# daihangpku/SW-NeRF

Measured on AMD Instinct MI355X. Metric: rays/sec (64+128 samples/ray), higher is better.
Workload: dtype f32

## Files before the change

### include/swnerf.h

```cpp
#ifndef SWNERF_H
#define SWNERF_H
#include <stddef.h>
#include <stdint.h>

#ifdef __cplusplus
extern "C" {
#endif

#define SWNERF_VERSION 112

#define SWNERF_E_ARG      (-1)
#define SWNERF_E_UNSUPP   (-2)

#define SWNERF_NET_CANON   0
#define SWNERF_NET_DNERF   1
#define SWNERF_NET_NOVIEW  2
#define SWNERF_NET_TNERF   3


int         swnerf_version(void);
const char* swnerf_last_error(void);

size_t swnerf_packed_floats(int kind);
int swnerf_pack_net(int kind, const float* const* params , int L_pos, int L_dir,
// ... 244 lines not shown
                         int64_t* count);
void swnerf_adam_caps(int* max_tensors, int* max_blocks, int64_t* chunk, size_t* descriptor_bytes);

#define SWNERF_PATCH_MAX_LEVELS 4
#define SWNERF_PATCH_MAX_SIDE   32
#define SWNERF_MULTIRES_LOSSES  11
int swnerf_patch_batch(int n_levels, const float* const* pyr_images , const int* level_hw , const double* focal ,
                       const int* corner , const int* patch , const float* images, int64_t n_images, const float* c2w,
                       const float* times, int64_t img_i, double near, double far, float* const* ray_batches ,
                       float* const* targets , float* full_patch, void* stream);
int swnerf_multires_loss(int n_levels, const int* patch_hw , const float* const* rgb ,
                         const float* const* rgb0 , const float* const* targets , const float* full_patch,
                         int add_global, float* losses, float* reconstructed, float* const* d_rgb ,
                         float* const* d_rgb0 , void* stream);

#ifdef __cplusplus
}
#endif
#endif
```

### sw-nerf_amd/csrc/pack_kernels.hip

```cpp
#include <hip/hip_runtime.h>
#include "../../include/swnerf.h"
#include "swnerf_common.h"
#include "host_util.h"

enum { KT_TRUNK = 0, KT_POS0 = 1, KT_POS1 = 2, KT_DIR = 3, KT_TIME = 4 };

struct PackSeg {
    const float* W; const float* b;
    float* dstW; float* dstB;
    int out_dim, in_dim;
    short NT, KT;
    short transpose, rowmap;
    int row0, kvalid;
    int max_steps;
    short kind;
    unsigned char ktype[10];
    short kbase[10];
};

#define PACK_MAX_SEGS 26
struct PackPlan { int n, Lp, Ld, Lt; int first_block[PACK_MAX_SEGS + 1]; PackSeg seg[PACK_MAX_SEGS]; };
static_assert(sizeof(PackPlan) <= 3800, "a pack plan must fit the kernel-argument segment");

__global__ void __launch_bounds__(256) pack_plan_kernel(PackPlan P) {
// ... 333 lines not shown
extern "C" int swnerf_pack_net_noview(const float* const* params, int L_pos, int out_ch, float* packed, void* stream) {
    if (!params || !packed) return sw_fail(SWNERF_E_ARG, "pack_net_noview: NULL pointer");
    if (L_pos < 0 || L_pos > 10) return sw_fail(SWNERF_E_UNSUPP, "pack_net_noview: %d position bands exceed 10", L_pos);
    if (out_ch < 4 || out_ch > SW_NOVIEW_MAX_OUT)
        return sw_fail(SWNERF_E_UNSUPP, "pack_net_noview: output_ch %d (the reference builds 4 or 5, nerf/run.py:231)", out_ch);
    for (int i = 0; i < 18; ++i) if (!params[i]) return sw_fail(SWNERF_E_ARG, "pack_net_noview: params[%d] is NULL", i);
    hipStream_t st = (hipStream_t)stream;
    Packer pk(st, packed, packed + SW_NOVIEW_W_FLOATS, L_pos, 0, 0);
    pk.trunk(params, params[16], params[17], out_ch, 3 * (1 + 2 * L_pos), 0);
    if (!pk.rc && (pk.w != packed + (size_t)SW_NOVIEW_STEPS * SW_STEP_FLOATS || pk.b != packed + SW_NOVIEW_W_FLOATS + SW_NOVIEW_BIAS_TILES(out_ch) * SW_BIAS_TILE_FLOATS))
        return sw_fail(SWNERF_E_ARG, "pack_net_noview: internal layout mismatch");
    pk.tail();
    return pk.flush();
}

extern "C" size_t swnerf_packed_bwd_floats_kind(int bwd_kind) {
    switch (bwd_kind) {
        case SWNERF_BWD_CANON: return (size_t)SW_BWD_FLOATS;
        case SWNERF_BWD_CANON_INPUT_GRAD: return (size_t)SW_BWD_IG_FLOATS;
        case SWNERF_BWD_DEFORM: return (size_t)SW_DBWD_FLOATS;
        case SWNERF_BWD_DNERF_FUSED: return (size_t)SW_BWD_DN_FLOATS;
    }
    return 0;
}

extern "C" int swnerf_pack_net_bwd_kind(int bwd_kind, const float* const* params, int L_pos, int L_dir, float* packed_bwd, void* stream) {
    if (!params || !packed_bwd) return sw_fail(SWNERF_E_ARG, "pack_net_bwd: NULL pointer");
    if (bwd_kind != SWNERF_BWD_CANON && bwd_kind != SWNERF_BWD_CANON_INPUT_GRAD && bwd_kind != SWNERF_BWD_DEFORM && bwd_kind != SWNERF_BWD_DNERF_FUSED)
        return sw_fail(SWNERF_E_ARG, "pack_net_bwd: unknown stream kind %d", bwd_kind);
    if (L_pos < 0 || L_pos > 10 || L_dir < 0 || L_dir > 4) return sw_fail(SWNERF_E_UNSUPP, "pack_net_bwd: embedder bands (%d,%d) exceed (10,4)", L_pos, L_dir);
// ... 64 lines not shown
```

### sw-nerf_amd/csrc/render_kernels.hip

```cpp
#include <hip/hip_runtime.h>
#include "../../include/swnerf.h"
#include "swnerf_common.h"
#include "mlp_core.h"
#include "host_util.h"
#include "mlp_kernels.h"

#include "render_pass.h"

struct QueryDev {
    const float* pts; int64_t M; const float* dirs; int64_t V; int shared;
    const float* w0; const float* b0; int nbias; const float* wvl; float* out;
};

__global__ void __launch_bounds__(256, 1) query_points_kernel(QueryDev P) {
    extern __shared__ __attribute__((aligned(16))) float lds_bias[];
    const int lane = threadIdx.x & 63, j = lane & 31, h = lane >> 5;
    const int wv = __builtin_amdgcn_readfirstlane(threadIdx.x >> 6);
    float* lds_ring = lds_bias + SW_LDS_BIAS_FLOATS + wv * SW_LDS_RING_FLOATS;
    float* lds_emb = lds_ring + SW_RING * SW_STEP_FLOATS;
    const int64_t tile = (int64_t)blockIdx.x * 4 + wv;
    bias_to_lds(lds_bias, P.b0, P.nbias);
    if (tile * 32 >= P.M) return;
    const int64_t row = tile * 32 + j;
    const bool live = row < P.M;
// ... 18 lines not shown
        ws.base = reinterpret_cast<const char*>(P.wvl);
        canon_tail_rows(in, demb, hv, lds_bias + h * 16, ws);
        float c3[3];
        head_valu<3, 4>(hv, ws, c3);
        sr += c3[0] + hb_rgb[1]; sg += c3[1] + hb_rgb[2]; sb += c3[2] + hb_rgb[3];
    }
    if (live && h == 0) {
        const float inv = 1.f / (float)nv;
        f32x4 r4 = {sr * inv, sg * inv, sb * inv, head[0]};
        *reinterpret_cast<f32x4*>(P.out + row * 4) = r4;
    }
}

int sw_tnerf_render_launch(const swnerf_pass_args& a, hipStream_t st);

extern "C" int swnerf_render_pass(const swnerf_pass_args* args, void* stream) {
    static const PassAccepts accepts = {"render_pass", {SW_COLS(11) | SW_COLS(12), SW_COLS(11) | SW_COLS(12), SW_COLS(8), ~0u },
        SWNERF_E_ARG, "%s: ray_batch must have 11 or 12 columns (use_viewdirs) or 8 (SWNERF_NET_NOVIEW), got %d for kind %d", true, 0};
    if (!args) return sw_fail(SWNERF_E_ARG, "render_pass: NULL args");
    const swnerf_pass_args& a = *args;
    if (a.kind < 0 || a.kind > SWNERF_NET_TNERF) return sw_fail(SWNERF_E_ARG, "unknown net kind %d", a.kind);
    int rc = pass_check(accepts, a);
    if (rc) return rc;
    if (a.kind == SWNERF_NET_TNERF) return sw_tnerf_render_launch(a, (hipStream_t)stream);
    const bool noview = a.kind == SWNERF_NET_NOVIEW;
    if (a.kind == SWNERF_NET_DNERF && a.cols != 12) return sw_fail(SWNERF_E_ARG, "render_pass: D-NeRF needs the frame_time column");
    if (noview && a.dx) return sw_fail(SWNERF_E_ARG, "render_pass: a static net has no position_delta output here");
    PassDev P = pass_dev(a);
    rc = noview ? stream_ptrs_noview(a.packed, a.out_ch, &P.w0, &P.b0, &P.nbias, &P.two_pass)
                : stream_ptrs(a.kind, a.packed, a.run_deform, &P.w0, &P.b0, &P.nbias, &P.two_pass);
    if (rc) return rc;
    P.dir_steps = noview ? 0 : SW_STEPS_DIR;
    P.time_steps = (a.kind == SWNERF_NET_DNERF && P.two_pass) ? SW_STEPS_TIME : 0;
    size_t lds = SW_LDS_FIXED_FLOATS * sizeof(float);
    if ((rc = pass_resampling(accepts.name, a, P, lds))) return rc;
    if (a.n_rays == 0) return 0;
    if (P.time_steps) {
        P.tb_off = (int)(lds / sizeof(float));
        lds += 4 * SW_TB_LDS_FLOATS * sizeof(float);
    }
    const dim3 grid((unsigned)((a.n_rays + 3) / 4)), block(256);
    hipStream_t st = (hipStream_t)stream;
    pass_startup_args(P, grid.x, noview ? SW_NOVIEW_STEPS : (a.kind == SWNERF_NET_DNERF && P.two_pass ? SW_DEFORM_STEPS + SW_CANON_STEPS : SW_CANON_STEPS));
    if (noview) hipLaunchKernelGGL((render_pass_kernel<false, false, 0, false>), grid, block, lds, st, P);
    else if (a.kind == SWNERF_NET_DNERF) hipLaunchKernelGGL(render_pass_kernel<true>, grid, block, lds, st, P);
    else {
        if (a.dx) {
            rc = sw_check(hipMemsetAsync(a.dx, 0, (size_t)a.n_rays * a.n_samples * 3 * sizeof(float), st), "render_pass dx fill");
            if (rc) return rc;
        }
        hipLaunchKernelGGL(render_pass_kernel<false>, grid, block, lds, st, P);
    }
    return sw_check(hipGetLastError(), "render_pass launch");
}

__global__ void __launch_bounds__(256) sample_coarse_kernel(swnerf_pass_args a, float* z_out, float* pts) {
    const int64_t idx = (int64_t)blockIdx.x * 256 + threadIdx.x;
    const int S = a.n_samples;
    if (idx >= a.n_rays * S) return;
    const int64_t ray = idx / S;
    const int s = (int)(idx - ray * S);
    const float* rb = a.ray_batch + ray * a.cols;
    const float z = z_sample(a, ray, rb[6], rb[7], s);
    z_out[idx] = z;
    if (pts) {
        pts[idx * 3 + 0] = rb[0] + rb[3] * z;
        pts[idx * 3 + 1] = rb[1] + rb[4] * z;
        pts[idx * 3 + 2] = rb[2] + rb[5] * z;
// ... 101 lines not shown
```

### sw-nerf_amd/csrc/render_pass.h

```cpp
#pragma once
#include <cstdlib>
#include "mlp_kernels.h"
#include "mlp_core_x3.h"
#include "resample.h"
#include "composite.h"

#define SW_LDS_SC 256
#define SW_LDS_SORT 1024
#define SW_LDS_WAVE_FLOATS (3 * SW_LDS_SC + SW_LDS_SORT)

struct PassDev {
    swnerf_pass_args a;
    const float* w0;
    const float* b0;
    int nbias;
    int two_pass;
    int sort_n, sort_s;
    float* act;
    float* bits;
    float* xs;
    float* act_d; float* bits_d; float* xs_d;
    int dir_steps;
    int time_steps;
    int tb_off;
    int warm_steps;
    int warm_blocks;
    int skew_mode;
    int skew_unit;
};

__device__ __forceinline__ float wave32_sum(float v) {
#pragma unroll
    for (int o = 16; o > 0; o >>= 1) v += __shfl_xor(v, o, 32);
    return v;
}

__device__ __forceinline__ float z_linear(const swnerf_pass_args& a, float near, float far, int s) {
    const float t = sw_linspace(0.f, 1.f, a.n_samples, s);
    if (!a.lindisp) return near * (1.f - t) + far * t;
    return 1.f / (1.f / near * (1.f - t) + 1.f / far * t);
}

__device__ __forceinline__ float z_sample(const swnerf_pass_args& a, int64_t ray, float near, float far, int s) {
// ... 171 lines not shown
    float* lds = PREC ? lds_all + X3Lds<DNERF>::FIXED + wv * SW_LDS_WAVE_FLOATS
                      : lds_all + PassLds<DNERF, TRAIN>::FIXED + wv * SW_LDS_WAVE_FLOATS;
    float* zc = lds;
    float* wc = lds + SW_LDS_SC;
    float* cdf = lds + 2 * SW_LDS_SC;
    float* srt = lds + 3 * SW_LDS_SC;

    const int S = a.n_samples;
    const bool resample = a.n_importance > 0;
    const float* rb = a.ray_batch + ray * a.cols;
    const float ox = rb[0], oy = rb[1], oz = rb[2], dx = rb[3], dy = rb[4], dz = rb[5];
    const float near = rb[6], far = rb[7];
    const float ft = (a.cols == 12) ? rb[8] : 0.f;
    const float v0 = VIEWS ? rb[a.cols - 3] : 0.f, v1 = VIEWS ? rb[a.cols - 2] : 0.f, v2 = VIEWS ? rb[a.cols - 1] : 0.f;
    const float dnorm = sqrtf(dx * dx + dy * dy + dz * dz);

    WStream ws;
    XStream xs;
    if constexpr (PREC != 0) {
        if (!DNERF) {
            f32x16 demb;
            pe_dir(v0, v1, v2, h, demb);
            tile_park(lds_dir, lane, demb);
        }
        x3_start(xs, reinterpret_cast<const char*>(P.w0), lds_bias, lds_ring, lane, wv);
    } else {
        ws_start(ws, P.w0, lds_bias, lds_ring, lane);
        if constexpr (VIEWS) {
            f32x16 demb;
            pe_dir(v0, v1, v2, h, demb);
            if constexpr (TRAIN) tile_park(lds_dir, lane, demb);
            view_bias_tile(demb, lds_vb, lane, ws);
        }
        if constexpr (DNERF) {
            if (P.time_steps) time_bias_tile(ft, h, lds_all + P.tb_off + wv * SW_TB_LDS_FLOATS, lane, ws);
        }
    }

    const float* zrow = a.z_vals ? a.z_vals + ray * S : nullptr;
    const float* zslot = PREC ? lds_x3w + X3Lds<DNERF>::DIR : lds_emb + SW_EMB_LDS_FLOATS;
    const unsigned zslot_addr = __builtin_amdgcn_readfirstlane((unsigned)(size_t)zslot);
    float pr = 0.f, pg = 0.f, pb = 0.f, pd = 0.f, pa = 0.f;
    double Tc = 1.0;
    const int ntiles = (S + 31) >> 5;
#pragma nounroll
    for (int tile = 0; tile < ntiles; ++tile) {
        const int s = tile * 32 + j;
// ... 118 lines not shown
            head[1] = 0.f; head[2] = 0.f;
            x3_canon_pipe<PREC>(px, py, pz, h, lds_dir, lane, head[0], rgb, xs);
            x3_rewind(xs, SW_X3_CANON_CHUNKS, lds_bias, lane);
        } else if constexpr (!VIEWS) {
            trunk_pass<false, false, false, true>(emb, lds_emb, 0.f, false, h, in, out, head, ws);
            float o5[5] = {0.f, 0.f, 0.f, 0.f, 0.f};
            const int nout = (a.out_ch == 5 && !a.raw) ? 4 : a.out_ch;
            head_valu_rt<8>(in, ws, nout, o5);
            ws.bias += (a.out_ch - nout) * 8 * SW_BIAS_TILE_FLOATS;
            rgb[0] = o5[0] + ws.bias[0]; rgb[1] = o5[1] + ws.bias[1]; rgb[2] = o5[2] + ws.bias[2];
            head[0] = o5[3] + ws.bias[3]; head[1] = 0.f; head[2] = 0.f;
            extra = o5[4] + ws.bias[4];
        } else {
            trunk_pass<false>(emb, lds_emb, 0.f, false, h, in, out, head, ws);
        }
        if (!TRAIN && PREC == 0 && VIEWS) canon_tail(in, lds_vb, rgb, ws.bias - SW_BIAS_TILE_FLOATS, ws);
        if constexpr (PREC == 0)
            ws_rewind(ws, P.w0 + (P.dir_steps + P.time_steps) * SW_STEP_FLOATS,
                      lds_bias + ((P.dir_steps ? SW_DIR_BIAS_TILES : 0) + (P.time_steps ? 8 : 0)) * SW_BIAS_TILE_FLOATS, lane);

        const float c0 = rgb[0], c1 = rgb[1], c2 = rgb[2];
        float sg = head[0];
        if (a.raw && live && h == 0) {
            if (!VIEWS && a.out_ch == 5) {
                float* o = a.raw + (ray * S + s) * 5;
                o[0] = c0; o[1] = c1; o[2] = c2; o[3] = sg; o[4] = extra;
            } else {
                f32x4 r4 = {c0, c1, c2, sg};
                *reinterpret_cast<f32x4*>(a.raw + (ray * S + s) * 4) = r4;
            }
        }
        if (a.noise) sg += a.noise[ray * S + sc];
        const float alpha = comp_alpha(sg, comp_dist(s + 1 < S, zn, z, dnorm), live);
        const float w = alpha * comp_transmittance(excl_cumprod_shfl<32>(comp_survival(alpha), j), Tc);
        if (live) {
            if (a.weights && h == 0) a.weights[ray * S + s] = w;
            if (a.z_out && h == 0) a.z_out[ray * S + s] = z;
            if (resample && h == 0) { zc[s] = z; wc[s] = w; }
        }
        comp_accumulate(w, c0, c1, c2, z, pr, pg, pb, pd, pa);
    }

    pr = wave32_sum(pr); pg = wave32_sum(pg); pb = wave32_sum(pb);
    pd = wave32_sum(pd); pa = wave32_sum(pa);
    if (lane == 0 && !ghost) comp_write_maps(pr, pg, pb, pd, pa, a.white_bkgd, ray, a.rgb_map, a.disp_map, a.acc_map, a.depth_map);
    if (!resample || ghost) return;

    wave_lds_sync();
    const int Ni = a.n_importance;
    const double sm = wave_sample_pdf(wc + 1, S - 1, MidBins{zc}, a.u ? a.u + ray * Ni : nullptr, Ni, cdf, srt, lane);
    if (a.z_std) {
        const float sd = wave_zstd(sm, srt, Ni, lane);
        if (lane == 0) a.z_std[ray] = sd;
    }
    wave_rank_merge(zc, S, P.sort_s, srt, Ni, P.sort_n, a.z_fine + ray * (S + Ni), lane);
}
```

### sw-nerf_amd/csrc/swnerf_common.h

```cpp
#pragma once
#include <math.h>
#include <stdint.h>

#if defined(__HIPCC__)
#define SW_HD __host__ __device__ __forceinline__
#else
#define SW_HD static inline
#endif

#define SW_STEP_FLOATS 256
#ifndef SW_RING
#define SW_RING 8
#endif
#define SW_TAIL 16
#define SW_BIAS_TILE_FLOATS 32

#define SW_STEPS_EMB    64
#define SW_STEPS_EMB_T  96
#define SW_STEPS_TIME   32
#define SW_STEPS_TRUNK  256
#define SW_STEPS_VIEWS  144
#define SW_STEPS_DIR    16
#define SW_STEPS_VIEWSH 128
#define SW_CANON_MAIN_STEPS (SW_STEPS_EMB + 4 * SW_STEPS_TRUNK + SW_STEPS_TRUNK + SW_STEPS_EMB + \
// ... 10 lines not shown
#define SW_NOVIEW_STEPS (SW_STEPS_EMB + 4 * SW_STEPS_TRUNK + SW_STEPS_TRUNK + SW_STEPS_EMB + 2 * SW_STEPS_TRUNK)
#define SW_NOVIEW_MAX_OUT 5
#define SW_NOVIEW_BIAS_TILES(out_ch) (64 + 8 * (out_ch) + 1)
#define SW_NOVIEW_W_FLOATS ((SW_NOVIEW_STEPS + SW_TAIL) * SW_STEP_FLOATS)
#define SW_NOVIEW_FLOATS (SW_NOVIEW_W_FLOATS + SW_NOVIEW_BIAS_TILES(SW_NOVIEW_MAX_OUT) * SW_BIAS_TILE_FLOATS)

#define SW_CANON_W_FLOATS   ((SW_CANON_STEPS + SW_TAIL) * SW_STEP_FLOATS)
#define SW_CANON_VL_OFFSET  (SW_CANON_W_FLOATS + SW_CANON_BIAS_TILES * SW_BIAS_TILE_FLOATS)
#define SW_CANON_VL_FLOATS  ((SW_STEPS_VIEWS + SW_TAIL) * SW_STEP_FLOATS)
#define SW_CANON_FOLD_OFFSET (SW_CANON_VL_OFFSET + SW_CANON_VL_FLOATS)
#define SW_CANON_FLOATS     (SW_CANON_FOLD_OFFSET + SW_FOLD_FLOATS)
#define SW_DNERF_W_FLOATS   ((SW_DEFORM_STEPS + SW_CANON_STEPS + SW_TAIL) * SW_STEP_FLOATS)
#define SW_DNERF_A_FLOATS   (SW_DNERF_W_FLOATS + (SW_DEFORM_BIAS_TILES + SW_CANON_BIAS_TILES) * SW_BIAS_TILE_FLOATS)
#define SW_DNERF_FLOATS     (SW_DNERF_A_FLOATS + SW_CANON_FLOATS)

#define SW_ACT_LD    2432
#define SW_ACT_HV    2304
#define SW_BWD_STEPS (16 + 128 + 7 * 256)
#define SW_BWD_W_FLOATS ((SW_BWD_STEPS + SW_TAIL) * SW_STEP_FLOATS)
#define SW_BWD_BIAS_TILES 8
#define SW_BWD_FLOATS (SW_BWD_W_FLOATS + SW_BWD_BIAS_TILES * SW_BIAS_TILE_FLOATS + SW_FOLD_FLOATS)
#define SW_BWD_IG_STEPS (SW_BWD_STEPS + 2 * 64)
#define SW_BWD_IG_W_FLOATS ((SW_BWD_IG_STEPS + SW_TAIL) * SW_STEP_FLOATS)
#define SW_BWD_IG_FLOATS (SW_BWD_IG_W_FLOATS + SW_BWD_BIAS_TILES * SW_BIAS_TILE_FLOATS + SW_FOLD_FLOATS)
#define SW_BWD_DN_STEPS (SW_BWD_IG_STEPS + 7 * 256)
#define SW_BWD_DN_W_FLOATS ((SW_BWD_DN_STEPS + SW_TAIL) * SW_STEP_FLOATS)
#define SW_BWD_DN_FLOATS (SW_BWD_DN_W_FLOATS + (SW_BWD_BIAS_TILES + 24) * SW_BIAS_TILE_FLOATS + SW_FOLD_FLOATS)
#define SW_DBWD_STEPS (7 * 256)
#define SW_DBWD_W_FLOATS ((SW_DBWD_STEPS + SW_TAIL) * SW_STEP_FLOATS)
#define SW_DBWD_BIAS_TILES 24
// ... 132 lines not shown
```

### sw-nerf_amd/swnerf/model.py

```python
import os
import torch
import torch.nn as nn
import torch.nn.functional as F
import numpy as np

from . import _lib, packing
from .embedder import img2mse, mse2psnr, to8b

_CANON_ORDER = ([f"pts_linears.{i}.{p}" for i in range(8) for p in ("weight", "bias")]
                + [f"{n}.{p}" for n in ("views_linears.0", "feature_linear", "alpha_linear", "rgb_linear")
                   for p in ("weight", "bias")])
_NOVIEW_ORDER = ([f"pts_linears.{i}.{p}" for i in range(8) for p in ("weight", "bias")]
                 + [f"output_linear.{p}" for p in ("weight", "bias")])
_DEFORM_ORDER = ([f"_time.{i}.{p}" for i in range(8) for p in ("weight", "bias")]
                 + [f"_time_out.{p}" for p in ("weight", "bias")])


def _bands(ch, d):
    if ch % d:
        return None
    q = ch // d - 1
    return q // 2 if q >= 0 and q % 2 == 0 else None


# ... 173 lines not shown
        buf = packing.pack_weights(self._pack_cache, "noview", _named(self, names), lambda L: L.swnerf_packed_floats(_lib.NET_NOVIEW),
                                   lambda L, arr, buf, st: L.swnerf_pack_net_noview(arr, Lp, out_ch, buf, st), "pack_net_noview")
        return buf, Lp, out_ch

    def packed_bwd_noview(self):
        names, Lp, out_ch = self._noview_params()
        return packing.pack_weights(self._pack_cache, "bwd_noview", _named(self, names), lambda L: L.swnerf_packed_bwd_noview_floats(),
                                    lambda L, arr, buf, st: L.swnerf_pack_net_bwd_noview(arr, Lp, out_ch, buf, st), "pack_net_bwd_noview")

    def packed(self):
        kind, names, Lp, Ld, Lt = self._pack_params()
        buf = packing.pack_weights(self._pack_cache, "fwd", _named(self, names), lambda L: L.swnerf_packed_floats(kind),
                                   lambda L, arr, buf, st: L.swnerf_pack_net(kind, arr, Lp, Ld, Lt, buf, st), "pack_net")
        return kind, buf, Lp, Ld, Lt

    def packed_x3(self):
        kind, packed, Lp, Ld, Lt = self.packed()
        buf = packing.pack_weights(self._pack_cache, "x3", _named(self, self._pack_params()[1]), lambda L: L.swnerf_packed_x3_floats_kind(kind),
                                   lambda L, arr, buf, st: L.swnerf_pack_net_x3_kind(kind, arr, Lp, Ld, Lt, _lib.ptr(packed), buf, st),
                                   "pack_net_x3")
        return buf, Lp, Ld

    def _forward_hip(self, x, t_emb=None, run_deform=0, want_dx=False):
        kind, packed, Lp, Ld, Lt = self.packed()
        x = _lib.dev_f32(x, "x", self.input_ch + self.input_ch_views)
        lead = x.shape[:-1]
        flat = x.reshape(-1, x.shape[-1])
        M = flat.shape[0]
        out = torch.empty((M, 4), dtype=torch.float32, device=x.device)
        dx = torch.empty((M, 3), dtype=torch.float32, device=x.device) if want_dx else None
# ... 205 lines not shown
```

### sw-nerf_amd/swnerf/parallel.py

```python
import os

import torch
import torch.distributed as dist

from .synth import shard_range


def gather_pixels(local, counts=None, group=None, force=False, async_op=False):
    if not (dist.is_available() and dist.is_initialized()):
        if force:
            raise RuntimeError("swnerf.parallel.gather_pixels(force=True) needs an initialised process group")
        return (local, None) if async_op else local
    if dist.get_world_size(group) == 1 and not force:
        return (local, None) if async_op else local
    world = dist.get_world_size(group)
    n, c = local.shape
    if counts is None:
        counts = [n] * world
    if all(k == counts[0] for k in counts):
        out = torch.empty((world * n, c), dtype=local.dtype, device=local.device)
        work = dist.all_gather_into_tensor(out, local.contiguous(), group=group, async_op=async_op)
        return (out, work) if async_op else out
    if async_op:
        raise ValueError("swnerf.parallel.gather_pixels: async_op needs equal shards")
# ... 25 lines not shown
    from . import render as _r, render_dnerf as _rd
    from .ray import get_rays_range
    n_streams = FRAME_STREAMS if streams is None else int(streams)

    def one(ray0, n):
        if frame_time is None:
            o, d = get_rays_range(H, W, K, c2w, ray0, n, device)
            rgb, disp, acc, _ = _r.render(H, W, K, chunk=chunk, rays=(o, d), **render_kwargs)
        else:
            focal = float(K[0][0]) if not isinstance(K, float) else K
            o, d = get_rays_range(H, W, focal, c2w, ray0, n, device)
            rgb, disp, acc, _ = _rd.render(H, W, focal, chunk=chunk, rays=(o, d), frame_time=frame_time, **render_kwargs)
        return torch.cat([rgb, disp[:, None], acc[:, None]], -1)

    def render_range(ray0, n):
        with torch.no_grad():
            dev = torch.device(device) if device is not None else None
            if n_streams <= 1 or n < 8192 or dev is None or dev.type != "cuda":
                return one(ray0, n)
            main = torch.cuda.current_stream(dev)
            if not any(p_.is_cuda for net in (render_kwargs.get("network_fn"), render_kwargs.get("network_fine")) if net is not None
                       for p_ in net.parameters()):
                return one(ray0, n)
            _r.prepack(render_kwargs.get("network_fn"), render_kwargs.get("network_fine"))
            key = (dev.index, n_streams)
            if key not in _FRAME_SIDE:
                _FRAME_SIDE[key] = [torch.cuda.Stream(device=dev) for _ in range(n_streams)]
            side = _FRAME_SIDE[key]
            ev0 = torch.cuda.Event()
            ev0.record(main)
            outs, a = [], 0
# ... 109 lines not shown
```

### sw-nerf_amd/swnerf/render.py

```python
import inspect
import os

import numpy as np
import torch

from . import _lib
from .ray import get_rays, sample_pdf, raw2outputs
from .embedder import EmbedFn, to8b
from .png import write_png
from .model import vallina_NeRF, NeRFOriginal, DirectTemporalNeRF

DEBUG = False
PASS_HOOK = None
Z_TAP = None


def batchify(fn, chunk):
    if chunk is None:
        return fn

    def ret(inputs):
        return torch.cat([fn(inputs[i:i + chunk]) for i in range(0, inputs.shape[0], chunk)], 0)
    return ret

# ... 72 lines not shown
_PRECISIONS = {"fp32": 0, "bf16x3": 3, "bf16x3-fine": 3, "bf16": 1}
_WARNED = {}
PRECISION = os.environ.get("SWNERF_PRECISION", "fp32")
if PRECISION not in _PRECISIONS:
    raise ValueError(f"swnerf: SWNERF_PRECISION={PRECISION!r} is not one of {sorted(_PRECISIONS)}")


def set_precision(name):
    global PRECISION
    if name not in _PRECISIONS:
        raise ValueError(f"swnerf.render.set_precision: unknown precision {name!r} (one of {sorted(_PRECISIONS)})")
    prev, PRECISION = PRECISION, name
    return prev


def prepack(*nets):
    for net in nets:
        if net is None or not hasattr(net, "packed"):
            continue
        if isinstance(net, vallina_NeRF) and net._noview_params() is not None:
            net.packed_noview()
        elif net._is_fused_arch():
            net.packed()
            if _PRECISIONS[PRECISION]:
                net.packed_x3()


def pass_args(rb, kind, packed, bands, S, out_ch, run_deform, inputs, outputs, n_importance=0, *, lindisp=False,
              white_bkgd=False, who="render_pass"):
    N, cols = rb.shape
    Ni = int(n_importance)
    a = _lib.PassArgs()
    a.ray_batch, a.n_rays, a.cols, a.kind, a.packed = rb.data_ptr(), N, cols, kind, packed.data_ptr()
    a.run_deform, (a.L_pos, a.L_dir, a.L_time), a.n_samples, a.out_ch = int(bool(run_deform)), bands, S, out_ch
    a.lindisp, a.white_bkgd, a.n_importance = int(bool(lindisp)), int(bool(white_bkgd)), Ni
    keep = [rb, packed]
    for name, t in inputs.items():
        if t is not None:
            t = _lib.dev_f32(t, name, Ni if name == "u" else S)
            if t.shape[0] != N:
                raise ValueError(f"swnerf.{who}: {name} must have {N} rows, got {tuple(t.shape)}")
            keep.append(t)
            setattr(a, name, t.data_ptr())
    shapes = {"rgb_map": (N, 3), "disp_map": (N,), "acc_map": (N,), "depth_map": (N,), "weights": (N, S), "raw": (N, S, out_ch),
              "dx": (N, S, 3), "z_out": (N, S), "z_fine": (N, S + Ni), "z_std": (N,)}
    out = {k: torch.empty(shapes[k], dtype=torch.float32, device=rb.device) for k in list(outputs) + (["z_fine", "z_std"] if Ni > 0 else [])}
    for k, t in out.items():
        setattr(a, k, t.data_ptr())
    return a, out, keep


def render_pass(ray_batch, net, n_samples, *, z_vals=None, lindisp=False, t_rand=None, noise=None, white_bkgd=False,
                want=("rgb_map", "disp_map", "acc_map"), n_importance=0, u=None, run_deform=True, precision=None):
    noview = isinstance(net, vallina_NeRF) and net._noview_params() is not None
    out_ch = 4
    if noview:
        packed, Lp, out_ch = net.packed_noview()
        kind, Ld, Lt, terms = _lib.NET_NOVIEW, 0, 0, 0
        if _PRECISIONS[PRECISION if precision is None else precision] and not _WARNED.get("noview_x3"):
            _WARNED["noview_x3"] = True
            import warnings
            warnings.warn(f"swnerf: precision {PRECISION if precision is None else precision!r} was requested, but the bf16 paths are built for the "
                          "nets WITH view directions only - this use_viewdirs=False net renders in fp32 (label your numbers accordingly)")
    else:
        kind, packed, Lp, Ld, Lt = net.packed()
        mode = PRECISION if precision is None else precision
        terms = _PRECISIONS[mode]
        if mode == "bf16x3-fine" and n_importance > 0:
            terms = 0
        if terms:
            packed, _, _ = net.packed_x3()
    rb = _lib.dev_f32(ray_batch, "ray_batch")
    N, S = rb.shape[0], int(n_samples)
    a, out, _keep = pass_args(rb, kind, packed, (Lp, Ld, Lt), S, out_ch, run_deform, dict(z_vals=z_vals, t_rand=t_rand, noise=noise, u=u),
                              want, n_importance, lindisp=lindisp, white_bkgd=white_bkgd)
    if PASS_HOOK is not None:
        PASS_HOOK("begin", N, S)
    if terms:
        _lib.check(_lib.lib().swnerf_render_pass_x3(a, terms, _lib.stream_of(rb)), "render_pass_x3")
    else:
        _lib.check(_lib.lib().swnerf_render_pass(a, _lib.stream_of(rb)), "render_pass")
    if PASS_HOOK is not None:
        PASS_HOOK("end", N, S)
    return out


def chunked_backward(rb, act_rows, div, widths, launch, gemm_jobs, rest_on_main=True):
    from .wgrad import _Fan, _chunk_gemms
    N = rb.shape[0]
    rows_per_ray = act_rows // N
    chunk = max(4, (TRAIN_BWD_CHUNK_ROWS // div // rows_per_ray) // 4 * 4)
    bufs = [torch.empty((min(N, chunk) * rows_per_ray, w), dtype=torch.float32, device=rb.device) for w in widths]
    fan = _Fan(rb.device)
# ... 160 lines not shown
    N = ray_batch.shape[0]
    t_rand, u, noise = _rng_inputs(N, N_samples, N_importance, perturb, raw_noise_std, pytest, ray_batch.device)
    S1 = N_samples + N_importance
    run_fn = network_fn if network_fine is None else network_fine
    if training:
        p0 = render_pass_train(ray_batch, network_fn, N_samples, lindisp=lindisp, t_rand=t_rand, noise=noise(N_samples),
                               white_bkgd=white_bkgd, n_importance=max(0, N_importance), u=u)
        if N_importance <= 0:
            return result_dict(p0, retraw)
        p1 = render_pass_train(ray_batch, run_fn, S1, z_vals=p0["z_fine"], noise=noise(S1), white_bkgd=white_bkgd)
        return result_dict(p1, retraw, p0, z_std=p0["z_std"])
    want = ["rgb_map", "disp_map", "acc_map"] + (["raw"] if (retraw and N_importance <= 0) else [])
    if N_importance <= 0:
        return result_dict(render_pass(ray_batch, network_fn, N_samples, lindisp=lindisp, t_rand=t_rand, noise=noise(N_samples),
                                       white_bkgd=white_bkgd, want=want), retraw)
    p0 = coarse_pass_resampled(ray_batch, network_fn, N_samples, N_importance, want=want, u=u, lindisp=lindisp, t_rand=t_rand,
                               noise=noise(N_samples), white_bkgd=white_bkgd)
    if Z_TAP is not None:
        Z_TAP["fused"] = p0["z_fine"]
    p1 = render_pass(ray_batch, run_fn, S1, z_vals=p0["z_fine"], noise=noise(S1), white_bkgd=white_bkgd,
                     want=["rgb_map", "disp_map", "acc_map"] + (["raw"] if retraw else []))
    return result_dict(p1, retraw, p0, z_std=p0["z_std"])


def result_dict(p, retraw, p0=None, **more):
    ret = {'rgb_map': p["rgb_map"], 'disp_map': p["disp_map"], 'acc_map': p["acc_map"]}
    z_std = more.pop("z_std", None)
    pd0 = more.pop("position_delta_0", None)
    ret.update({k: v for k, v in more.items() if v is not None})
    if retraw:
        ret['raw'] = p["raw"]
    if p0 is not None:
        ret['rgb0'], ret['disp0'], ret['acc0'] = p0["rgb_map"], p0["disp_map"], p0["acc_map"]
    if pd0 is not None:
        ret['position_delta_0'] = pd0
    if z_std is not None:
        ret['z_std'] = z_std
# ... 144 lines not shown
        if pending is not None:
            done(pending)
        pending = (i, h_rgb, h_disp, ev)
    if pending is not None:
        done(pending)


def render_path(render_poses, hwf, K, chunk, render_kwargs, gt_imgs=None, savedir=None, render_factor=0):
    H, W, focal = hwf
    if render_factor != 0:
        H, W, focal = H // render_factor, W // render_factor, focal / render_factor
    rgbs, disps = [], []

    def frames():
        for i, c2w in enumerate(render_poses):
            rgb, disp, acc, _ = render(H, W, K, chunk=chunk, c2w=c2w[:3, :4], **render_kwargs)
            yield i, rgb, disp

    def consume(i, rgb, disp):
        rgbs.append(rgb)
        disps.append(disp)
        if gt_imgs is not None and render_factor == 0:
            gt = gt_imgs[i]
            gt = gt.cpu().numpy() if isinstance(gt, torch.Tensor) else np.asarray(gt)
            print(-10. * np.log10(np.mean(np.square(rgb - gt))))
        if savedir is not None:
            write_png(os.path.join(savedir, '{:03d}.png'.format(i)), to8b(rgb))
    pipelined_frames(frames(), consume)
    return np.stack(rgbs, 0), np.stack(disps, 0)
```

### sw-nerf_amd/swnerf/render_dnerf.py

```python
import contextvars
import os

import numpy as np
import torch

from . import _lib
from .embedder import to8b
from .png import write_png
from .ray import get_rays, sample_pdf, raw2outputs
from .render import (fused_plan, render_pass, render_pass_train, pack_ray_batch, _rng_inputs, _coarse_z, coarse_pass_resampled,
                     pipelined_frames, sample_coarse, wants_grad, result_dict, batchify_rays_with, image_outputs, pass_args,
                     chunked_backward, f32_grads, ray_ptrs, TRAIN_FUSED_MAX_SAMPLES)
from .model import DirectTemporalNeRF, NeRFOriginal

DEBUG = False
DNERF_CHUNK_DIV = int(os.environ.get("SWNERF_DNERF_CHUNK_DIV", "2"))


def batchify(fn, chunk):
    if chunk is None:
        return fn

    def ret(inputs_pos, inputs_time):
        outs, dxs = [], []
# ... 129 lines not shown
        if runs_deform(net, t0):
            p = _render_pass_train_dnerf(ray_batch, net, S, z_vals=z_in, lindisp=lindisp, t_rand=tr, noise=nz, white_bkgd=white_bkgd)
            return p, p["z"], p["dx"]
        canon = net._occ if isinstance(net, DirectTemporalNeRF) else net
        p = render_pass_train(ray_batch, canon, S, z_vals=z_in, lindisp=lindisp, t_rand=tr, noise=nz, white_bkgd=white_bkgd)
        if z_in is None:
            with torch.no_grad():
                z_in = sample_coarse(ray_batch.detach(), S, lindisp, tr)
        return p, z_in, torch.zeros((N, S, 3), dtype=torch.float32, device=ray_batch.device)

    z_std = p0t = pd0 = None
    if z_vals is None and N_importance > 0:
        nz0 = noise(N_samples)
        with torch.no_grad():
            p0 = render_pass(ray_batch.detach(), network_fn, N_samples, lindisp=lindisp, t_rand=t_rand, noise=nz0,
                             white_bkgd=white_bkgd, want=[], n_importance=N_importance, u=u, run_deform=runs_deform(network_fn, t0))
        if use_two_models_for_fine:
            p0t, _, pd0 = train_pass(network_fn, N_samples, None, t_rand, nz0)
        z_in, z_std, t_rand = p0["z_fine"], p0["z_std"], None
    else:
        z_in = None if z_vals is None else _lib.dev_f32(z_vals, "z_vals")
        if z_in is not None:
            t_rand = None
    p1, z_final, pd = train_pass(run_fn, S1, z_in, t_rand, noise(S1))
    return result_dict(p1, retraw, p0t, z_vals=z_final, position_delta=pd, position_delta_0=pd0, z_std=z_std)


def render_rays(ray_batch, network_fn, network_query_fn, N_samples, retraw=False, lindisp=False, perturb=0.,
                N_importance=0, network_fine=None, white_bkgd=False, raw_noise_std=0., verbose=False, pytest=False,
                z_vals=None, use_two_models_for_fine=False):
    plan = None
# ... 13 lines not shown
    t0 = _single_time(ray_batch)
    t_rand, u, noise = _rng_inputs(N, N_samples, N_importance, perturb, raw_noise_std, pytest, ray_batch.device)
    run_fn = network_fn if network_fine is None else network_fine
    full = ["rgb_map", "disp_map", "acc_map", "dx"]
    z_std = None
    p0 = None
    if z_vals is None:
        if N_importance <= 0:
            p1 = render_pass(ray_batch, run_fn, N_samples, lindisp=lindisp, t_rand=t_rand, noise=noise(N_samples),
                             white_bkgd=white_bkgd, want=full + ["z_out"] + (["raw"] if retraw else []),
                             run_deform=runs_deform(run_fn, t0))
            z_final = p1["z_out"]
        else:
            want0 = ["rgb_map", "disp_map", "acc_map", "dx"] if use_two_models_for_fine else []
            p0 = coarse_pass_resampled(ray_batch, network_fn, N_samples, N_importance, want=want0, u=u, lindisp=lindisp,
                                       t_rand=t_rand, noise=noise(N_samples), white_bkgd=white_bkgd, run_deform=runs_deform(network_fn, t0))
            z_final, z_std = p0["z_fine"], p0["z_std"]
            p1 = None
    else:
        z_final = _lib.dev_f32(z_vals, "z_vals")
        p1 = None
    if p1 is None:
        S1 = z_final.shape[-1]
        p1 = render_pass(ray_batch, run_fn, S1, z_vals=z_final, noise=noise(S1), white_bkgd=white_bkgd,
                         want=full + (["raw"] if retraw else []), run_deform=runs_deform(run_fn, t0))
    p0_own = p0 if (p0 is not None and use_two_models_for_fine) else None
    return result_dict(p1, retraw, p0_own, z_vals=z_final, position_delta=p1["dx"],
                       position_delta_0=None if p0_own is None else p0_own["dx"], z_std=z_std)


def _render_rays_unfused(ray_batch, network_fn, network_query_fn, N_samples, retraw, lindisp, perturb, N_importance,
# ... 1 lines not shown
    N_rays = ray_batch.shape[0]
    rays_o, rays_d = ray_batch[:, 0:3], ray_batch[:, 3:6]
    viewdirs = ray_batch[:, -3:] if ray_batch.shape[-1] > 9 else None
    bounds = torch.reshape(ray_batch[..., 6:9], [-1, 1, 3])
    near, far, frame_time = bounds[..., 0], bounds[..., 1], bounds[..., 2]
    z_samples = None
    rgb_map_0 = disp_map_0 = acc_map_0 = position_delta_0 = None
    fused_coarse = None
    if z_vals is None and N_importance > 0 and not use_two_models_for_fine and ray_batch.shape[-1] == 12:
        with torch.no_grad():
            if fused_plan(network_query_fn, [network_fn], need_time=True) is not None:
                t0 = _single_time(ray_batch)
                t_rand, u, noise = _rng_inputs(N_rays, N_samples, N_importance, perturb, raw_noise_std, pytest, ray_batch.device)
                fused_coarse = coarse_pass_resampled(ray_batch.detach(), network_fn, N_samples, N_importance, want=[], u=u,
                                                     lindisp=lindisp, t_rand=t_rand, noise=noise(N_samples), white_bkgd=white_bkgd,
                                                     run_deform=runs_deform(network_fn, t0))
    z_std = None
    if fused_coarse is not None:
        z_vals, z_std = fused_coarse["z_fine"], fused_coarse["z_std"]
    elif z_vals is None:
        z_vals = _coarse_z(near, far, N_rays, N_samples, lindisp, perturb, pytest, ray_batch)
        pts = rays_o[..., None, :] + rays_d[..., None, :] * z_vals[..., :, None]
        if N_importance > 0:
            if use_two_models_for_fine:
                raw, position_delta_0 = network_query_fn(pts, viewdirs, frame_time, network_fn)
                rgb_map_0, disp_map_0, acc_map_0, weights, _ = raw2outputs(raw, z_vals, rays_d, raw_noise_std, white_bkgd, pytest=pytest)
            else:
                with torch.no_grad():
                    raw, _ = network_query_fn(pts, viewdirs, frame_time, network_fn)
                    _, _, _, weights, _ = raw2outputs(raw, z_vals, rays_d, raw_noise_std, white_bkgd, pytest=pytest)
            z_vals_mid = .5 * (z_vals[..., 1:] + z_vals[..., :-1])
# ... 70 lines not shown
```

Baseline: 547,600.

## Skip view-dependent RGB tail in coarse pass when only resampling weights are needed

Adds a trunk-only packed weight layout and a resample entry point so the coarse pass can run just the density trunk when no coarse maps are requested. The view-direction embedding, RGB tail and compositing sums are skipped, and the color inputs are zeroed. Only the density weights feed importance sampling. This removes the view-branch matmuls from the coarse pass, at the cost of a separately packed and cached weight buffer and new code paths gated by a context variable.

```diff
diff --git a/include/swnerf.h b/include/swnerf.h
--- a/include/swnerf.h
+++ b/include/swnerf.h
@@ -282,6 +282,10 @@
                          int add_global, float* losses, float* reconstructed, float* const* d_rgb ,
                          float* const* d_rgb0 , void* stream);
 
+size_t swnerf_packed_trunk_floats(int kind);
+int swnerf_pack_net_trunk(int kind, const float* const* params , int L_pos, int L_time, float* packed_trunk, void* stream);
+int swnerf_render_pass_resample(const swnerf_pass_args* args , const float* packed_trunk, void* stream);
+
 #ifdef __cplusplus
 }
 #endif
diff --git a/sw-nerf_amd/csrc/pack_kernels.hip b/sw-nerf_amd/csrc/pack_kernels.hip
--- a/sw-nerf_amd/csrc/pack_kernels.hip
+++ b/sw-nerf_amd/csrc/pack_kernels.hip
@@ -371,6 +371,38 @@
     return pk.flush();
 }
 
+extern "C" size_t swnerf_packed_trunk_floats(int kind) {
+    return kind == SWNERF_NET_CANON ? (size_t)SW_TRUNK_FLOATS : kind == SWNERF_NET_DNERF ? (size_t)SW_TRUNK_DNERF_FLOATS : 0;
+}
+
+extern "C" int swnerf_pack_net_trunk(int kind, const float* const* params, int L_pos, int L_time, float* packed_trunk, void* stream) {
+    if (!params || !packed_trunk) return sw_fail(SWNERF_E_ARG, "pack_net_trunk: NULL pointer");
+    if (kind != SWNERF_NET_CANON && kind != SWNERF_NET_DNERF) return sw_fail(SWNERF_E_ARG, "pack_net_trunk: unknown kind %d", kind);
+    if (L_pos < 0 || L_pos > 10 || L_time < 0 || L_time > 10)
+        return sw_fail(SWNERF_E_UNSUPP, "pack_net_trunk: embedder bands (%d,%d) exceed (10,10)", L_pos, L_time);
+    const int np = kind == SWNERF_NET_CANON ? 24 : 42;
+    for (int i = 0; i < np; ++i) if (!params[i]) return sw_fail(SWNERF_E_ARG, "pack_net_trunk: params[%d] is NULL", i);
+    const int Cpos = 3 * (1 + 2 * L_pos), Ctime = 1 + 2 * L_time;
+    hipStream_t st = (hipStream_t)stream;
+    if (kind == SWNERF_NET_DNERF) {
+        Packer pk(st, packed_trunk, packed_trunk + SW_TRUNK_DNERF_W_FLOATS, L_pos, 0, L_time);
+        pk.trunk(params + 24, params[40], params[41], 3, Cpos, Ctime);
+        pk.trunk(params, params[20], params[21], 1, Cpos, 0, params[23], 3);
+        if (!pk.rc && (pk.w != packed_trunk + (size_t)(SW_DEFORM_STEPS + SW_TRUNK_STEPS) * SW_STEP_FLOATS || pk.b != packed_trunk + SW_TRUNK_DNERF_A_FLOATS))
+            return sw_fail(SWNERF_E_ARG, "pack_net_trunk: internal layout mismatch");
+        pk.tail();
+        int rc = pk.flush();
+        if (rc) return rc;
+        packed_trunk += SW_TRUNK_DNERF_A_FLOATS;
+    }
+    Packer pk(st, packed_trunk, packed_trunk + SW_TRUNK_W_FLOATS, L_pos, 0, 0);
+    pk.trunk(params, params[20], params[21], 1, Cpos, 0, params[23], 3);
+    if (!pk.rc && (pk.w != packed_trunk + (size_t)SW_TRUNK_STEPS * SW_STEP_FLOATS || pk.b != packed_trunk + SW_TRUNK_FLOATS))
+        return sw_fail(SWNERF_E_ARG, "pack_net_trunk: internal layout mismatch");
+    pk.tail();
+    return pk.flush();
+}
+
 extern "C" size_t swnerf_packed_bwd_floats_kind(int bwd_kind) {
     switch (bwd_kind) {
         case SWNERF_BWD_CANON: return (size_t)SW_BWD_FLOATS;
diff --git a/sw-nerf_amd/csrc/render_kernels.hip b/sw-nerf_amd/csrc/render_kernels.hip
--- a/sw-nerf_amd/csrc/render_kernels.hip
+++ b/sw-nerf_amd/csrc/render_kernels.hip
@@ -56,7 +56,7 @@
 
 int sw_tnerf_render_launch(const swnerf_pass_args& a, hipStream_t st);
 
-extern "C" int swnerf_render_pass(const swnerf_pass_args* args, void* stream) {
+static int render_pass_launch(const swnerf_pass_args* args, const float* packed_trunk, void* stream) {
     static const PassAccepts accepts = {"render_pass", {SW_COLS(11) | SW_COLS(12), SW_COLS(11) | SW_COLS(12), SW_COLS(8), ~0u },
         SWNERF_E_ARG, "%s: ray_batch must have 11 or 12 columns (use_viewdirs) or 8 (SWNERF_NET_NOVIEW), got %d for kind %d", true, 0};
     if (!args) return sw_fail(SWNERF_E_ARG, "render_pass: NULL args");
@@ -74,6 +74,16 @@
     if (rc) return rc;
     P.dir_steps = noview ? 0 : SW_STEPS_DIR;
     P.time_steps = (a.kind == SWNERF_NET_DNERF && P.two_pass) ? SW_STEPS_TIME : 0;
+    int steps = noview ? SW_NOVIEW_STEPS : (P.two_pass ? SW_DEFORM_STEPS + SW_CANON_STEPS : SW_CANON_STEPS);
+    if (packed_trunk && !noview && a.n_importance > 0 && !a.rgb_map && !a.disp_map && !a.acc_map && !a.depth_map && !a.weights && !a.raw && !a.dx && !a.z_out) {
+        const float* t = (a.kind == SWNERF_NET_DNERF && !P.two_pass) ? packed_trunk + SW_TRUNK_DNERF_A_FLOATS : packed_trunk;
+        P.weights_only = 1;
+        P.w0 = t;
+        P.b0 = t + (P.two_pass ? SW_TRUNK_DNERF_W_FLOATS : SW_TRUNK_W_FLOATS);
+        P.nbias = ((P.two_pass ? SW_DEFORM_BIAS_TILES : 0) + SW_TRUNK_BIAS_TILES) * SW_BIAS_TILE_FLOATS;
+        P.dir_steps = 0;
+        steps = (P.two_pass ? SW_DEFORM_STEPS : 0) + SW_TRUNK_STEPS;
+    }
     size_t lds = SW_LDS_FIXED_FLOATS * sizeof(float);
     if ((rc = pass_resampling(accepts.name, a, P, lds))) return rc;
     if (a.n_rays == 0) return 0;
@@ -83,7 +93,7 @@
     }
     const dim3 grid((unsigned)((a.n_rays + 3) / 4)), block(256);
     hipStream_t st = (hipStream_t)stream;
-    pass_startup_args(P, grid.x, noview ? SW_NOVIEW_STEPS : (a.kind == SWNERF_NET_DNERF && P.two_pass ? SW_DEFORM_STEPS + SW_CANON_STEPS : SW_CANON_STEPS));
+    pass_startup_args(P, grid.x, steps);
     if (noview) hipLaunchKernelGGL((render_pass_kernel<false, false, 0, false>), grid, block, lds, st, P);
     else if (a.kind == SWNERF_NET_DNERF) hipLaunchKernelGGL(render_pass_kernel<true>, grid, block, lds, st, P);
     else {
@@ -94,6 +104,12 @@
         hipLaunchKernelGGL(render_pass_kernel<false>, grid, block, lds, st, P);
     }
     return sw_check(hipGetLastError(), "render_pass launch");
+}
+
+extern "C" int swnerf_render_pass(const swnerf_pass_args* args, void* stream) { return render_pass_launch(args, nullptr, stream); }
+
+extern "C" int swnerf_render_pass_resample(const swnerf_pass_args* args, const float* packed_trunk, void* stream) {
+    return render_pass_launch(args, packed_trunk, stream);
 }
 
 __global__ void __launch_bounds__(256) sample_coarse_kernel(swnerf_pass_args a, float* z_out, float* pts) {
diff --git a/sw-nerf_amd/csrc/render_pass.h b/sw-nerf_amd/csrc/render_pass.h
--- a/sw-nerf_amd/csrc/render_pass.h
+++ b/sw-nerf_amd/csrc/render_pass.h
@@ -27,6 +27,7 @@
     int warm_blocks;
     int skew_mode;
     int skew_unit;
+    int weights_only;
 };
 
 __device__ __forceinline__ float wave32_sum(float v) {
@@ -228,6 +229,7 @@
     const float ft = (a.cols == 12) ? rb[8] : 0.f;
     const float v0 = VIEWS ? rb[a.cols - 3] : 0.f, v1 = VIEWS ? rb[a.cols - 2] : 0.f, v2 = VIEWS ? rb[a.cols - 1] : 0.f;
     const float dnorm = sqrtf(dx * dx + dy * dy + dz * dz);
+    const bool wonly = !TRAIN && PREC == 0 && VIEWS && P.weights_only;
 
     WStream ws;
     XStream xs;
@@ -241,10 +243,12 @@
     } else {
         ws_start(ws, P.w0, lds_bias, lds_ring, lane);
         if constexpr (VIEWS) {
-            f32x16 demb;
-            pe_dir(v0, v1, v2, h, demb);
-            if constexpr (TRAIN) tile_park(lds_dir, lane, demb);
-            view_bias_tile(demb, lds_vb, lane, ws);
+            if (!wonly) {
+                f32x16 demb;
+                pe_dir(v0, v1, v2, h, demb);
+                if constexpr (TRAIN) tile_park(lds_dir, lane, demb);
+                view_bias_tile(demb, lds_vb, lane, ws);
+            }
         }
         if constexpr (DNERF) {
             if (P.time_steps) time_bias_tile(ft, h, lds_all + P.tb_off + wv * SW_TB_LDS_FLOATS, lane, ws);
@@ -393,7 +397,10 @@
         } else {
             trunk_pass<false>(emb, lds_emb, 0.f, false, h, in, out, head, ws);
         }
-        if (!TRAIN && PREC == 0 && VIEWS) canon_tail(in, lds_vb, rgb, ws.bias - SW_BIAS_TILE_FLOATS, ws);
+        if constexpr (!TRAIN && PREC == 0 && VIEWS) {
+            if (!wonly) canon_tail(in, lds_vb, rgb, ws.bias - SW_BIAS_TILE_FLOATS, ws);
+            else rgb[0] = rgb[1] = rgb[2] = 0.f;
+        }
         if constexpr (PREC == 0)
             ws_rewind(ws, P.w0 + (P.dir_steps + P.time_steps) * SW_STEP_FLOATS,
                       lds_bias + ((P.dir_steps ? SW_DIR_BIAS_TILES : 0) + (P.time_steps ? 8 : 0)) * SW_BIAS_TILE_FLOATS, lane);
@@ -417,12 +424,14 @@
             if (a.z_out && h == 0) a.z_out[ray * S + s] = z;
             if (resample && h == 0) { zc[s] = z; wc[s] = w; }
         }
-        comp_accumulate(w, c0, c1, c2, z, pr, pg, pb, pd, pa);
-    }
-
-    pr = wave32_sum(pr); pg = wave32_sum(pg); pb = wave32_sum(pb);
-    pd = wave32_sum(pd); pa = wave32_sum(pa);
-    if (lane == 0 && !ghost) comp_write_maps(pr, pg, pb, pd, pa, a.white_bkgd, ray, a.rgb_map, a.disp_map, a.acc_map, a.depth_map);
+        if (!wonly) comp_accumulate(w, c0, c1, c2, z, pr, pg, pb, pd, pa);
+    }
+
+    if (!wonly) {
+        pr = wave32_sum(pr); pg = wave32_sum(pg); pb = wave32_sum(pb);
+        pd = wave32_sum(pd); pa = wave32_sum(pa);
+    }
+    if (lane == 0 && !ghost && !wonly) comp_write_maps(pr, pg, pb, pd, pa, a.white_bkgd, ray, a.rgb_map, a.disp_map, a.acc_map, a.depth_map);
     if (!resample || ghost) return;
 
     wave_lds_sync();
diff --git a/sw-nerf_amd/csrc/swnerf_common.h b/sw-nerf_amd/csrc/swnerf_common.h
--- a/sw-nerf_amd/csrc/swnerf_common.h
+++ b/sw-nerf_amd/csrc/swnerf_common.h
@@ -48,6 +48,14 @@
 #define SW_DNERF_A_FLOATS   (SW_DNERF_W_FLOATS + (SW_DEFORM_BIAS_TILES + SW_CANON_BIAS_TILES) * SW_BIAS_TILE_FLOATS)
 #define SW_DNERF_FLOATS     (SW_DNERF_A_FLOATS + SW_CANON_FLOATS)
 
+#define SW_TRUNK_STEPS SW_NOVIEW_STEPS
+#define SW_TRUNK_BIAS_TILES (64 + 8 + 1)
+#define SW_TRUNK_W_FLOATS ((SW_TRUNK_STEPS + SW_TAIL) * SW_STEP_FLOATS)
+#define SW_TRUNK_FLOATS (SW_TRUNK_W_FLOATS + SW_TRUNK_BIAS_TILES * SW_BIAS_TILE_FLOATS)
+#define SW_TRUNK_DNERF_W_FLOATS ((SW_DEFORM_STEPS + SW_TRUNK_STEPS + SW_TAIL) * SW_STEP_FLOATS)
+#define SW_TRUNK_DNERF_A_FLOATS (SW_TRUNK_DNERF_W_FLOATS + (SW_DEFORM_BIAS_TILES + SW_TRUNK_BIAS_TILES) * SW_BIAS_TILE_FLOATS)
+#define SW_TRUNK_DNERF_FLOATS (SW_TRUNK_DNERF_A_FLOATS + SW_TRUNK_FLOATS)
+
 #define SW_ACT_LD    2432
 #define SW_ACT_HV    2304
 #define SW_BWD_STEPS (16 + 128 + 7 * 256)
diff --git a/sw-nerf_amd/swnerf/model.py b/sw-nerf_amd/swnerf/model.py
--- a/sw-nerf_amd/swnerf/model.py
+++ b/sw-nerf_amd/swnerf/model.py
@@ -211,6 +211,11 @@
                                    lambda L, arr, buf, st: L.swnerf_pack_net(kind, arr, Lp, Ld, Lt, buf, st), "pack_net")
         return kind, buf, Lp, Ld, Lt
 
+    def packed_trunk(self):
+        kind, names, Lp, Ld, Lt = self._pack_params()
+        return packing.pack_weights(self._pack_cache, "trunk", _named(self, names), lambda L: L.swnerf_packed_trunk_floats(kind),
+                                    lambda L, arr, buf, st: L.swnerf_pack_net_trunk(kind, arr, Lp, Lt, buf, st), "pack_net_trunk")
+
     def packed_x3(self):
         kind, packed, Lp, Ld, Lt = self.packed()
         buf = packing.pack_weights(self._pack_cache, "x3", _named(self, self._pack_params()[1]), lambda L: L.swnerf_packed_x3_floats_kind(kind),
diff --git a/sw-nerf_amd/swnerf/parallel.py b/sw-nerf_amd/swnerf/parallel.py
--- a/sw-nerf_amd/swnerf/parallel.py
+++ b/sw-nerf_amd/swnerf/parallel.py
@@ -63,7 +63,7 @@
         return torch.cat([rgb, disp[:, None], acc[:, None]], -1)
 
     def render_range(ray0, n):
-        with torch.no_grad():
+        with torch.no_grad(), _r.coarse_weights_only():
             dev = torch.device(device) if device is not None else None
             if n_streams <= 1 or n < 8192 or dev is None or dev.type != "cuda":
                 return one(ray0, n)
diff --git a/sw-nerf_amd/swnerf/render.py b/sw-nerf_amd/swnerf/render.py
--- a/sw-nerf_amd/swnerf/render.py
+++ b/sw-nerf_amd/swnerf/render.py
@@ -1,3 +1,5 @@
+import contextlib
+import contextvars
 import inspect
 import os
 
@@ -110,6 +112,25 @@
     return prev
 
 
+_COARSE_WEIGHTS_ONLY = contextvars.ContextVar("swnerf_coarse_weights_only", default=False)
+
+
+@contextlib.contextmanager
+def coarse_weights_only(on=True):
+    token = _COARSE_WEIGHTS_ONLY.set(bool(on))
+    try:
+        yield
+    finally:
+        _COARSE_WEIGHTS_ONLY.reset(token)
+
+
+def weights_only_applies(net, N_samples, N_importance, precision=None):
+    mode = PRECISION if precision is None else precision
+    terms = 0 if mode == "bf16x3-fine" else _PRECISIONS[mode]
+    noview = isinstance(net, vallina_NeRF) and net._noview_params() is not None
+    return N_importance > 0 and not terms and not noview and pass_can_resample(N_samples, N_importance)
+
+
 def prepack(*nets):
     for net in nets:
         if net is None or not hasattr(net, "packed"):
@@ -120,6 +141,8 @@
             net.packed()
             if _PRECISIONS[PRECISION]:
                 net.packed_x3()
+            if _COARSE_WEIGHTS_ONLY.get():
+                net.packed_trunk()
 
 
 def pass_args(rb, kind, packed, bands, S, out_ch, run_deform, inputs, outputs, n_importance=0, *, lindisp=False,
@@ -147,7 +170,7 @@
 
 
 def render_pass(ray_batch, net, n_samples, *, z_vals=None, lindisp=False, t_rand=None, noise=None, white_bkgd=False,
-                want=("rgb_map", "disp_map", "acc_map"), n_importance=0, u=None, run_deform=True, precision=None):
+                want=("rgb_map", "disp_map", "acc_map"), n_importance=0, u=None, run_deform=True, precision=None, weights_only=False):
     noview = isinstance(net, vallina_NeRF) and net._noview_params() is not None
     out_ch = 4
     if noview:
@@ -170,9 +193,12 @@
     N, S = rb.shape[0], int(n_samples)
     a, out, _keep = pass_args(rb, kind, packed, (Lp, Ld, Lt), S, out_ch, run_deform, dict(z_vals=z_vals, t_rand=t_rand, noise=noise, u=u),
                               want, n_importance, lindisp=lindisp, white_bkgd=white_bkgd)
+    trunk = net.packed_trunk() if (weights_only and not list(want) and not noview and not terms and n_importance > 0) else None
     if PASS_HOOK is not None:
         PASS_HOOK("begin", N, S)
-    if terms:
+    if trunk is not None:
+        _lib.check(_lib.lib().swnerf_render_pass_resample(a, _lib.ptr(trunk), _lib.stream_of(rb)), "render_pass_resample")
+    elif terms:
         _lib.check(_lib.lib().swnerf_render_pass_x3(a, terms, _lib.stream_of(rb)), "render_pass_x3")
     else:
         _lib.check(_lib.lib().swnerf_render_pass(a, _lib.stream_of(rb)), "render_pass")
@@ -363,13 +389,14 @@
     if N_importance <= 0:
         return result_dict(render_pass(ray_batch, network_fn, N_samples, lindisp=lindisp, t_rand=t_rand, noise=noise(N_samples),
                                        white_bkgd=white_bkgd, want=want), retraw)
-    p0 = coarse_pass_resampled(ray_batch, network_fn, N_samples, N_importance, want=want, u=u, lindisp=lindisp, t_rand=t_rand,
-                               noise=noise(N_samples), white_bkgd=white_bkgd)
+    skip0 = _COARSE_WEIGHTS_ONLY.get() and weights_only_applies(network_fn, N_samples, N_importance)
+    p0 = coarse_pass_resampled(ray_batch, network_fn, N_samples, N_importance, want=[] if skip0 else want, u=u, lindisp=lindisp,
+                               t_rand=t_rand, noise=noise(N_samples), white_bkgd=white_bkgd, weights_only=skip0)
     if Z_TAP is not None:
         Z_TAP["fused"] = p0["z_fine"]
     p1 = render_pass(ray_batch, run_fn, S1, z_vals=p0["z_fine"], noise=noise(S1), white_bkgd=white_bkgd,
                      want=["rgb_map", "disp_map", "acc_map"] + (["raw"] if retraw else []))
-    return result_dict(p1, retraw, p0, z_std=p0["z_std"])
+    return result_dict(p1, retraw, None if skip0 else p0, z_std=p0["z_std"])
 
 
 def result_dict(p, retraw, p0=None, **more):
@@ -544,7 +571,8 @@
 
     def frames():
         for i, c2w in enumerate(render_poses):
-            rgb, disp, acc, _ = render(H, W, K, chunk=chunk, c2w=c2w[:3, :4], **render_kwargs)
+            with coarse_weights_only():
+                rgb, disp, acc, _ = render(H, W, K, chunk=chunk, c2w=c2w[:3, :4], **render_kwargs)
             yield i, rgb, disp
 
     def consume(i, rgb, disp):
diff --git a/sw-nerf_amd/swnerf/render_dnerf.py b/sw-nerf_amd/swnerf/render_dnerf.py
--- a/sw-nerf_amd/swnerf/render_dnerf.py
+++ b/sw-nerf_amd/swnerf/render_dnerf.py
@@ -167,7 +167,8 @@
         nz0 = noise(N_samples)
         with torch.no_grad():
             p0 = render_pass(ray_batch.detach(), network_fn, N_samples, lindisp=lindisp, t_rand=t_rand, noise=nz0,
-                             white_bkgd=white_bkgd, want=[], n_importance=N_importance, u=u, run_deform=runs_deform(network_fn, t0))
+                             white_bkgd=white_bkgd, want=[], n_importance=N_importance, u=u, run_deform=runs_deform(network_fn, t0),
+                             weights_only=True)
         if use_two_models_for_fine:
             p0t, _, pd0 = train_pass(network_fn, N_samples, None, t_rand, nz0)
         z_in, z_std, t_rand = p0["z_fine"], p0["z_std"], None
@@ -211,7 +212,8 @@
         else:
             want0 = ["rgb_map", "disp_map", "acc_map", "dx"] if use_two_models_for_fine else []
             p0 = coarse_pass_resampled(ray_batch, network_fn, N_samples, N_importance, want=want0, u=u, lindisp=lindisp,
-                                       t_rand=t_rand, noise=noise(N_samples), white_bkgd=white_bkgd, run_deform=runs_deform(network_fn, t0))
+                                       t_rand=t_rand, noise=noise(N_samples), white_bkgd=white_bkgd, run_deform=runs_deform(network_fn, t0),
+                                       weights_only=not use_two_models_for_fine)
             z_final, z_std = p0["z_fine"], p0["z_std"]
             p1 = None
     else:
@@ -243,7 +245,7 @@
                 t_rand, u, noise = _rng_inputs(N_rays, N_samples, N_importance, perturb, raw_noise_std, pytest, ray_batch.device)
                 fused_coarse = coarse_pass_resampled(ray_batch.detach(), network_fn, N_samples, N_importance, want=[], u=u,
                                                      lindisp=lindisp, t_rand=t_rand, noise=noise(N_samples), white_bkgd=white_bkgd,
-                                                     run_deform=runs_deform(network_fn, t0))
+                                                     run_deform=runs_deform(network_fn, t0), weights_only=True)
     z_std = None
     if fused_coarse is not None:
         z_vals, z_std = fused_coarse["z_fine"], fused_coarse["z_std"]
```

Result: no change. 545,500 (-0.4%).
